# hjr37/diff-gaussian-rasterization

Measured on AMD Instinct MI355X. Metric: Mviews/sec fwd+bwd @1080p, 500k Gaussians, higher is better.
Workload: dtype f32

## Files before the change

### diff-gaussian-rasterization_amd/csrc/render_common.h

```cpp
#pragma once
#include "dgr_common.h"
#include "kernels.h"
#include "wave_reduce.h"
#include "exact_math.h"

namespace dgr {

__device__ __forceinline__ uint4 blend_slot(const uint4* __restrict__ sched, const uint2* __restrict__ ranges,
                                            const uint32_t* __restrict__ sched_flag, int tiles, bool* overflowed = nullptr,
                                            bool* quadrant_lists = nullptr) {
    const int flag = __builtin_amdgcn_readfirstlane((int)*sched_flag);
    if (overflowed) *overflowed = (flag & 2) != 0;
    if (quadrant_lists) *quadrant_lists = (flag & 4) != 0;
    if (flag & 1) return sched[blockIdx.x];
    const int tile = xcd_contiguous((int)blockIdx.x, tiles);
    const uint2 r = ranges[tile];
    return make_uint4((uint32_t)tile, r.x, r.y, 0u);
}

__device__ __forceinline__ bool wave_any(bool p) { return __builtin_amdgcn_ballot_w64(p) != 0ull; }

namespace {

constexpr float LOG2E = 1.4426950408889634f, LN2 = 0.6931471805599453f;
constexpr float ALPHA_MIN = 15.0f / 255.0f;

enum { ALPHA_REF = 0, ALPHA_FAST = 1, ALPHA_GLIBC = 2 };
template <int AM>
struct AlphaPath {
    static constexpr bool LOG2 = (AM == ALPHA_FAST);
    static constexpr float PSCALE = LOG2 ? LOG2E : 1.0f;
    static constexpr float PUNSCALE = LOG2 ? LN2 : 1.0f;
    static constexpr bool TABLE = (AM == ALPHA_GLIBC);
};
template <int AM, bool UNTESTED_ARG = false>
__device__ __forceinline__ float alpha_raw(float o, float p2, const uint64_t* tab) {
    if (AM == ALPHA_FAST) return o * __builtin_amdgcn_exp2f(p2);
    if (AM == ALPHA_GLIBC) return o * exp_glibc<UNTESTED_ARG>(p2, tab);
    return o * exp_p32<UNTESTED_ARG>(p2);
}
template <int AM>
__device__ __forceinline__ float t_div(float T, float om, float& inv) {
    if (AM == ALPHA_FAST) { inv = __builtin_amdgcn_rcpf(om); return T * inv; }
    return div_ref(T, om, inv);
}

template <int NB, typename LIST_T = unsigned short, int NLISTS = 4, bool KEEP_ID = true>
struct StagedT {
    typedef LIST_T list_t;
    static constexpr bool HAS_ID = KEEP_ID;
    static constexpr int SLOTS = NB;
    static constexpr int SENTINEL = NB;
    static constexpr int LIST_LD = NB + 8;
    static constexpr int REC_BYTES = 32;
    float4 rec[2 * (NB + 1)];
    float4 rgbd[NB + 1];
    uint32_t id[KEEP_ID ? NB : 1];
    LIST_T list[NLISTS][LIST_LD];
    int cnt4[4][NLISTS];
};
using Staged = StagedT<DGR_TILE_PIX>;

template <int AM>
__device__ __forceinline__ void gather_record(const float4* __restrict__ rec, uint32_t gid, float4& staged0, float4& q0, float4& q1, float4& q2) {
    constexpr float PSCALE = AlphaPath<AM>::PSCALE;
    q0 = rec[DGR_REC_STRIDE * (size_t)gid + 0];
    q1 = rec[DGR_REC_STRIDE * (size_t)gid + 1];
    q2 = rec[DGR_REC_STRIDE * (size_t)gid + 2];
    staged0 = make_float4(q0.x, q0.y, -0.5f * PSCALE * q1.x, -0.5f * PSCALE * q1.z);
}

template <bool HALF_CODES>
__device__ __forceinline__ unsigned reach_code(const float4& q0, const float4& q1, float l2, float tile_x0, float tile_y0);

template <int AM, bool HALF_CODES = false, class S>
__device__ __forceinline__ unsigned stage_one(S& s, int slot, uint32_t gid, const float4* __restrict__ rec,
                                              float tile_x0, float tile_y0) {
    float4 q0, q1, q2;
    gather_record<AM>(rec, gid, s.rec[2 * slot], q0, q1, q2);
    const float o = q0.w;
    const float l2 = __log2f(o * (255.0f / 15.0f));
    constexpr float PSCALE = AlphaPath<AM>::PSCALE;
    float lthr = (o > 0.f) ? (-l2 * (AlphaPath<AM>::LOG2 ? 1.0f : LN2) - 1.0e-4f) : 3.0e38f;
    float zword = __int_as_float(slot);
    if (HALF_CODES) {
        lthr = fmaxf(lthr, -3.0e38f);
        lthr = __int_as_float(((__float_as_int(lthr) + 0xFF) & ~0xFF) | slot);
        zword = 0.f;
    }
    s.rec[2 * slot + 1] = make_float4(-PSCALE * q1.y, o, zword, lthr);
    s.rgbd[slot] = make_float4(q2.x, q2.y, q2.z, q0.z);
    if (S::HAS_ID) s.id[slot] = gid;
    return reach_code<HALF_CODES>(q0, q1, l2, tile_x0, tile_y0);
}
template <bool HALF_CODES>
__device__ __forceinline__ unsigned reach_code(const float4& q0, const float4& q1, float l2, float tile_x0, float tile_y0) {
    const float tau = 2.0f * 0.6931471805599453f * l2;
    const float det = q1.x * q1.z - q1.y * q1.y;
    if (!(tau > 0.0f)) return 0u;
    if (!(det > 0.0f && q1.x > 0.0f && q1.z > 0.0f)) return HALF_CODES ? 0xFFu : 0xFu;
    const float k = tau * __builtin_amdgcn_rcpf(det);
    const float hx = __builtin_amdgcn_sqrtf(k * q1.z) * 1.001f + 0.05f, hy = __builtin_amdgcn_sqrtf(k * q1.x) * 1.001f + 0.05f;
    const float gx = q0.x - tile_x0, gy = q0.y - tile_y0;
    const bool xl = (gx + hx >= 0.0f) && (gx - hx <= 7.0f), xr = (gx + hx >= 8.0f) && (gx - hx <= 15.0f);
    if (HALF_CODES) {
        const float lo = gy - hy, hi = gy + hy;
        const unsigned xm = (xl ? 0x33u : 0u) | (xr ? 0xCCu : 0u);
        const unsigned ym = ((hi >= 0.0f) && (lo <= 3.0f) ? 0x05u : 0u) | ((hi >= 4.0f) && (lo <= 7.0f) ? 0x0Au : 0u) |
                            ((hi >= 8.0f) && (lo <= 11.0f) ? 0x50u : 0u) | ((hi >= 12.0f) && (lo <= 15.0f) ? 0xA0u : 0u);
        return xm & ym;
    }
    const bool yt = (gy + hy >= 0.0f) && (gy - hy <= 7.0f), yb = (gy + hy >= 8.0f) && (gy - hy <= 15.0f);
    return (xl && yt ? 1u : 0u) | (xr && yt ? 2u : 0u) | (xl && yb ? 4u : 0u) | (xr && yb ? 8u : 0u);
}

constexpr int TAG_SHIFT = DGR_TAG_SHIFT;
constexpr uint32_t ID_MASK = DGR_ID_MASK;
enum { TAGS_BYTES_QUADRANT = 1, TAGS_BYTES_HALVES = 2 };

__device__ __forceinline__ uint8_t* half_tags(const uint32_t* point_list, const uint32_t* sched_flag) {
    return carve_binning(reinterpret_cast<char*>(const_cast<uint32_t*>(point_list)), (size_t)sched_flag[-1]).pair_cov;
}
__device__ __forceinline__ uint32_t spread4(uint32_t c) { return (c & 1u) | ((c & 2u) << 1) | ((c & 4u) << 2) | ((c & 8u) << 3); }
__device__ __forceinline__ uint32_t fold8(uint32_t t) {
    t = (t | (t >> 1)) & 0x55u;
    return (t & 1u) | ((t >> 1) & 2u) | ((t >> 2) & 4u) | ((t >> 3) & 8u);
}

__device__ __forceinline__ uint32_t pack4(uint32_t w) { return (w & 1u) | ((w >> 7) & 2u) | ((w >> 14) & 4u) | ((w >> 21) & 8u); }
__device__ __forceinline__ uint32_t tag_byte(uint32_t up, uint32_t lo) { return spread4(pack4(up)) | (spread4(pack4(lo)) << 1); }

template <int AM, int TAGS, class S>
__device__ __forceinline__ unsigned stage_tagged(S& s, int slot, uint32_t entry, const float4* __restrict__ rec,
                                                 const uint8_t* __restrict__ tag8) {
    constexpr float PSCALE = AlphaPath<AM>::PSCALE;
    unsigned code = (unsigned)*tag8;
    if (code == 0u) return 0u;
    if (TAGS == TAGS_BYTES_QUADRANT) code = fold8(code);
    const uint32_t gid = entry & ID_MASK;
    float4 q0, q1, q2;
    gather_record<AM>(rec, gid, s.rec[2 * slot], q0, q1, q2);
    s.rec[2 * slot + 1] = make_float4(-PSCALE * q1.y, q0.w, __int_as_float(slot * 4), __int_as_float(slot * 16));
    s.rgbd[slot] = make_float4(q2.x, q2.y, q2.z, q0.z);
    s.id[slot] = gid;
    return code;
}

__device__ __forceinline__ uint2* live_list(const uint32_t* point_list, const uint32_t* sched_flag) {
    return reinterpret_cast<uint2*>(carve_binning(reinterpret_cast<char*>(const_cast<uint32_t*>(point_list)), (size_t)sched_flag[-1]).pair_keys);
}

template <int NB, int NLISTS = 4>
struct StagedLiveT {
    typedef uint32_t list_t;
    static constexpr bool HAS_ID = true;
    static constexpr int SLOTS = NB;
    static constexpr int SENTINEL = NB;
    static constexpr int LIST_LD = NB + 8;
    static constexpr int REC_BYTES = 48;
    float4 rec[3 * (NB + 1)];
    uint32_t id[NB];
    uint32_t list[NLISTS][LIST_LD];
    int cnt4[4][NLISTS];
};

template <int AM, bool QUADRANT, class S>
__device__ __forceinline__ unsigned stage_live(S& s, int slot, uint2 e, const float4* __restrict__ rec) {
    constexpr float PSCALE = AlphaPath<AM>::PSCALE;
    unsigned code = e.y & 0xFFu;
    if (QUADRANT) code = fold8(code);
    const uint32_t gid = e.x & ID_MASK;
    float4 q0, q1, q2;
    gather_record<AM>(rec, gid, s.rec[3 * slot], q0, q1, q2);
    s.rec[3 * slot + 1] = make_float4(-PSCALE * q1.y, q0.w, __int_as_float(slot * 4), __int_as_float((int)(e.y >> 8)));
    s.rec[3 * slot + 2] = make_float4(q2.x, q2.y, q2.z, q0.z);
    s.id[slot] = gid;
    return code;
}
template <class S>
__device__ __forceinline__ void write_sentinel_live(S& s) {
    constexpr int NB = S::SLOTS;
    s.rec[3 * NB] = make_float4(0.f, 0.f, 0.f, 0.f);
    s.rec[3 * NB + 1] = make_float4(0.f, 0.f, __int_as_float(NB * 4), __int_as_float(0x7fffffff));
    s.rec[3 * NB + 2] = make_float4(0.f, 0.f, 0.f, 0.f);
}

__device__ __forceinline__ int lanes_below(unsigned long long m) {
    return (int)__builtin_amdgcn_mbcnt_hi((unsigned)(m >> 32), __builtin_amdgcn_mbcnt_lo((unsigned)m, 0u));
}

template <class S>
__device__ __forceinline__ int build_lists(S& s, unsigned code, int tid, int wave, int lane) {
    typedef typename S::list_t LT;
    unsigned long long bal[4];
#pragma unroll
    for (int w = 0; w < 4; w++) {
        bal[w] = __ballot((code >> w) & 1u);
        if (lane == 0) s.cnt4[wave][w] = __popcll(bal[w]);
    }
    __syncthreads();
#pragma unroll
    for (int w = 0; w < 4; w++) {
        if ((code >> w) & 1u) {
            int base = 0;
            for (int sw = 0; sw < wave; sw++) base += s.cnt4[sw][w];
            s.list[w][base + lanes_below(bal[w])] = (LT)(tid * S::REC_BYTES);
        }
    }
    const int n = __builtin_amdgcn_readfirstlane(s.cnt4[0][wave] + s.cnt4[1][wave] + s.cnt4[2][wave] + s.cnt4[3][wave]);
    __syncthreads();
    if (lane < 4) s.list[wave][n + lane] = (LT)(S::SENTINEL * S::REC_BYTES);
    return n;
}

template <class S>
__device__ __forceinline__ int build_half_lists(S& s, unsigned code, int tid, int wave, int lane) {
    typedef typename S::list_t LT;
    unsigned long long bal[8];
#pragma unroll
    for (int l = 0; l < 8; l++) {
        bal[l] = __ballot((code >> l) & 1u);
        if (lane == 0) s.cnt4[wave][l] = __popcll(bal[l]);
    }
    __syncthreads();
    int before = 0, all = 0;
    if (lane < 8) {
#pragma unroll
        for (int sw = 0; sw < 4; sw++) {
            const int c = s.cnt4[sw][lane];
            before += sw < wave ? c : 0;
            all += c;
        }
    }
#pragma unroll
    for (int l = 0; l < 8; l++) {
        const int base = __builtin_amdgcn_readlane(before, l);
        if ((code >> l) & 1u) s.list[l][base + lanes_below(bal[l])] = (LT)(tid * S::REC_BYTES);
    }
    const int l0 = 2 * wave;
    const int n0 = __builtin_amdgcn_readlane(all, l0), n1 = __builtin_amdgcn_readlane(all, l0 + 1);
    __syncthreads();
    const int n = max(n0, n1);
    for (int i = n0 + lane; i < n + 4; i += 64) s.list[l0][i] = (LT)(S::SENTINEL * S::REC_BYTES);
    for (int i = n1 + lane; i < n + 4; i += 64) s.list[l0 + 1][i] = (LT)(S::SENTINEL * S::REC_BYTES);
    return n;
}

template <class S>
__device__ __forceinline__ int build_paired_lists(S& s, unsigned code8, int tid, int wave, int lane, unsigned long long (&split)[2]) {
    typedef typename S::list_t LT;
    static_assert(sizeof(LT) == 4 && S::SLOTS <= 128, "paired lists: 32-bit entries, at most two ranks per lane");
    unsigned long long bal[4];
#pragma unroll
    for (int w = 0; w < 4; w++) {
        bal[w] = __ballot(((code8 >> (2 * w)) & 3u) != 0u);
        if (lane == 0) s.cnt4[wave][w] = __popcll(bal[w]);
    }
    __syncthreads();
    int before = 0, all = 0;
    if (lane < 4) {
#pragma unroll
        for (int sw = 0; sw < 4; sw++) {
            const int c = s.cnt4[sw][lane];
            before += sw < wave ? c : 0;
            all += c;
        }
    }
#pragma unroll
    for (int w = 0; w < 4; w++) {
        const unsigned t = (code8 >> (2 * w)) & 3u;
        const int base = __builtin_amdgcn_readlane(before, w);
        if (t != 0u) s.list[2 * w][base + lanes_below(bal[w])] = (LT)(tid * S::REC_BYTES) | t;
    }
    const int n = __builtin_amdgcn_readlane(all, wave);
    __syncthreads();
    LT* const LU = s.list[2 * wave];
    LT* const LL = s.list[2 * wave + 1];
    if (n <= 64) {
        const bool have = lane < n;
        const unsigned e0 = have ? LU[lane] : 0u;
        const int t0 = (int)(e0 & 3u);
        const int tm1 = __builtin_amdgcn_update_dpp(0, t0, 0x138, 0xf, 0xf, true);
        const int tm2 = __builtin_amdgcn_update_dpp(0, tm1, 0x138, 0xf, 0xf, true);
        const int tp1 = __builtin_amdgcn_update_dpp(0, t0, 0x130, 0xf, 0xf, true);
        const int tp2 = __builtin_amdgcn_update_dpp(0, tp1, 0x130, 0xf, 0xf, true);
        const bool odd = (lane & 1) != 0;
        const bool a_self = odd ? (tm1 * t0 == 2) : (t0 * tp1 == 2);
        const bool a_side = odd ? (tp1 * tp2 == 2) : (tm2 * tm1 == 2);
        const bool p2 = !a_self && !a_side && (odd ? (t0 * tp1 == 2) : (tm1 * t0 == 2));
        const bool first = odd ? p2 : a_self, second = odd ? a_self : p2;
        const unsigned long long keep = __ballot(have && !second);
        const int steps = __popcll(keep);
        if (have) {
            const int st = lanes_below(keep) - (second ? 1 : 0);
            const LT o = e0 & ~3u;
            if (first || second) {
                (t0 == 1 ? LU : LL)[st] = o;
            } else {
                LU[st] = o;
                LL[st] = o;
            }
        }
        if (lane < 4) {
            LU[steps + lane] = (LT)(S::SENTINEL * S::REC_BYTES);
            LL[steps + lane] = (LT)(S::SENTINEL * S::REC_BYTES);
        }
        split[0] = __ballot(lane < steps && LU[lane] != LL[lane]);
        split[1] = 0ull;
        return steps;
    }
    const LT ea = lane < n ? LU[lane] : 0u, eb = lane + 64 < n ? LU[lane + 64] : 0u;
    if (lane < n) { LU[lane] = ea & ~3u; LL[lane] = ea & ~3u; }
    if (lane + 64 < n) { LU[lane + 64] = eb & ~3u; LL[lane + 64] = eb & ~3u; }
    if (lane < 4) {
        LU[n + lane] = (LT)(S::SENTINEL * S::REC_BYTES);
        LL[n + lane] = (LT)(S::SENTINEL * S::REC_BYTES);
    }
    split[0] = split[1] = 0ull;
    return n;
}
// ... 159 lines not shown
```

### diff-gaussian-rasterization_amd/csrc/render_light.hip

```cpp
#include "render_common.h"

namespace dgr {
namespace {

constexpr int FWD_UNROLL = 2;

template <bool HALVES>
struct StagedFwd {
    typedef StagedT<DGR_TILE_PIX, unsigned short, HALVES ? 8 : 4, !HALVES> staged_t;
    staged_t f;
    float unc[DGR_TILE_PIX];
    uint32_t cnt[DGR_TILE_PIX];
    uint32_t hit[DGR_TILE_PIX];
    alignas(16) uint32_t live4[4];
    uint64_t exptab[32];
};

template <class SF>
__device__ __forceinline__ uint32_t flush_slot(SF& sf, const RenderFwdLightArgs& a, uint8_t* tag8, uint2* live, uint32_t list0, uint32_t pos0,
                                               uint32_t live_base, int tid, bool staged) {
    uint32_t t8 = 0u;
    if (staged) {
        if constexpr (!SF::staged_t::HAS_ID) {
            t8 = tag_byte(sf.hit[tid], __float_as_uint(sf.f.rec[2 * tid + 1].z));
        } else {
            t8 = spread4(pack4(sf.hit[tid])) * 3u;
        }
        tag8[list0 + pos0 + tid] = (uint8_t)t8;
    }
    const unsigned long long bal = __ballot(t8 != 0u);
    if ((tid & 63) == 0) sf.live4[tid >> 6] = (uint32_t)__popcll(bal);
    __syncthreads();
    const uint4 c = *reinterpret_cast<const uint4*>(sf.live4);
    if (t8 != 0u) {
        const int wave = tid >> 6;
        const uint32_t before = (wave > 0 ? c.x : 0u) + (wave > 1 ? c.y : 0u) + (wave > 2 ? c.z : 0u);
        uint32_t gid;
        if constexpr (SF::staged_t::HAS_ID) gid = sf.f.id[tid];
        else gid = a.point_list[list0 + pos0 + tid];
        live[list0 + live_base + before + (uint32_t)lanes_below(bal)] = make_uint2(gid, ((pos0 + (uint32_t)tid) << 8) | t8);
        if (sf.cnt[tid] != 0u) {
            atomicAdd(&a.gau_uncertainty[gid], sf.unc[tid]);
            atomicAdd(&a.gau_related_pixels[gid], (int)sf.cnt[tid]);
        }
    }
    return live_base + (uint32_t)__builtin_amdgcn_readfirstlane((int)(c.x + c.y + c.z + c.w));
}

template <int AM, bool HALVES>
__device__ __forceinline__ void render_fwd_light_body(const RenderFwdLightArgs& a, StagedFwd<HALVES>& sf, const uint4 slot, const bool overflowed) {
    typename StagedFwd<HALVES>::staged_t& s = sf.f;
    const int tile = (int)slot.x;
    const int tid = threadIdx.x, wave = tid >> 6, lane = tid & 63;
    const auto [tx, ty, px, py, inside, pix_id] = tile_pixel(tile, a.grid_x, a.W, a.H, wave, lane);
    const f2 pxy = {(float)px, (float)py};
    const float tile_x0 = (float)(tx * DGR_BLOCK_X), tile_y0 = (float)(ty * DGR_BLOCK_Y);
    const int my_list = HALVES ? 2 * wave + (lane >> 5) : wave;
    uint8_t* const tag8 = half_tags(a.point_list, a.sched_flag);
    uint2* const live = live_list(a.point_list, a.sched_flag);
    uint32_t live_base = 0;
    unsigned char* const mark_base = (HALVES && lane >= 32) ? reinterpret_cast<unsigned char*>(&s.rec[1].z) + wave
                                                             : reinterpret_cast<unsigned char*>(sf.hit) + wave;
    const int mark_stride = (HALVES && lane >= 32) ? 32 : 4;

    const uint2 range = make_uint2(slot.y, slot.z);
    const int total = (int)(range.y - range.x);

    float T = 1.0f, C0 = 0.f, C1 = 0.f, C2 = 0.f, weight = 0.f, Dd = 0.f, D_median = 0.f;
    uint32_t last_contributor = 0;
    float ub = inside ? 0.f : -__builtin_inff();
    const float gt_px = inside ? a.gt_depth[pix_id] : 0.f;
    if (tid == 0) write_sentinel(s);
    if (AlphaPath<AM>::TABLE) exp_ref_table_fill(sf.exptab, tid);
    bool have_flush = false;
    int last_base = 0;

    for (int base = 0; base < total; base += DGR_TILE_PIX) {
        if (__syncthreads_and(ub < 0.f)) break;
        last_base = base;
        if (have_flush) live_base = flush_slot(sf, a, tag8, live, range.x, (uint32_t)(base - DGR_TILE_PIX), live_base, tid, true);
        sf.unc[tid] = 0.f;
        sf.cnt[tid] = 0u;
        sf.hit[tid] = 0u;
        have_flush = true;
        const int cnt = min(DGR_TILE_PIX, total - base);
        unsigned code = 0;
        if (tid < cnt) code = stage_one<AM, HALVES>(s, tid, a.point_list[range.x + base + tid], a.rec, tile_x0, tile_y0);
        const int n = HALVES ? build_half_lists(s, code, tid, wave, lane) : build_lists(s, code, tid, wave, lane);

        for (int k = 0; k < n; k += FWD_UNROLL) {
            float4 q0[FWD_UNROLL], q1[FWD_UNROLL];
            load2(s, my_list, k, q0, q1);
#pragma unroll
            for (int u = 0; u < FWD_UNROLL; u++) {
                f2 dxy;
                const float p2 = pair_p2<AM>(q0[u], q1[u], pxy, dxy);
                if ((p2 <= ub) & (p2 >= q1[u].w)) {
                  const float alpha = fminf(0.99f, alpha_raw<AM>(q1[u].y, p2, sf.exptab));
                  if (alpha >= ALPHA_MIN) {
#pragma clang fp contract(off)
                    const float test_T = T * (1.0f - alpha);
                    if (test_T < 0.0001f) {
                        ub = -__builtin_inff();
                    } else {
                        const int j = HALVES ? (__float_as_int(q1[u].w) & 0xFF) : __float_as_int(q1[u].z);
                        const float4 cd = s.rgbd[j];
                        mark_base[j * mark_stride] = 1;
                        const float w = alpha * T;
                        C0 = __builtin_fmaf(cd.x, w, C0); C1 = __builtin_fmaf(cd.y, w, C1); C2 = __builtin_fmaf(cd.z, w, C2);
                        weight = weight + w;
                        Dd = __builtin_fmaf(cd.w, w, Dd);
                        if (T > 0.5f && test_T < 0.5f) {
                            D_median = cd.w;
                            const float e = cd.w - gt_px;
                            atomicAdd(&sf.unc[j], e * e * w);
                            atomicAdd(&sf.cnt[j], 1u);
                        }
                        T = test_T;
                        last_contributor = (uint32_t)(base + j + 1);
                    }
                  }
                }
            }
            if (!wave_any(ub >= 0.f)) break;
        }
    }
    __syncthreads();
    if (have_flush) live_base = flush_slot(sf, a, tag8, live, range.x, (uint32_t)last_base, live_base, tid, tid < total - last_base);
    if (tid == 0) a.live_counts[tile] = live_base;
    for (int p = (have_flush ? last_base + DGR_TILE_PIX : 0) + tid; p < total; p += DGR_TILE_PIX) tag8[range.x + p] = 0;

    if (overflowed) {
        C0 = C1 = C2 = weight = Dd = D_median = __builtin_nanf("");
    }
    if (inside) {
        const uint32_t N = (uint32_t)a.W * (uint32_t)a.H;
        a.n_contrib[pix_id] = last_contributor;
        a.out_color[pix_id] = C0 + T * a.bg[0];
        a.out_color[N + pix_id] = C1 + T * a.bg[1];
        a.out_color[2 * N + pix_id] = C2 + T * a.bg[2];
        a.out_alpha[pix_id] = weight;
        a.out_depth[pix_id] = Dd;
        a.out_median[pix_id] = D_median;
        a.out_depth_var[pix_id] = 0.0f;
    }
}

template <int AM>
__global__ void __launch_bounds__(256, 8) render_fwd_light_kernel(RenderFwdLightArgs a) {
    __shared__ union { StagedFwd<true> h; StagedFwd<false> q; } sf;
    if (a.rep.host && blockIdx.x == 0 && threadIdx.x == 0) report_status(a.rep, a.status);
    bool overflowed, quadrant_lists;
    const uint4 slot = blend_slot(a.sched, a.ranges, a.sched_flag, a.grid_x * a.grid_y, &overflowed, &quadrant_lists);
    if (quadrant_lists) render_fwd_light_body<AM, false>(a, sf.q, slot, overflowed);
    else render_fwd_light_body<AM, true>(a, sf.h, slot, overflowed);
}

constexpr int NACC_LIGHT = 14;

struct BwdTailLight {
    uint64_t exptab[32];
};
template <bool DET, bool HALVES = false, bool ABS = false>
using StagedBwd = BwdBatch<StagedLiveT<bwd_batch_entries(DET), HALVES ? 8 : 4>, NACC_LIGHT, DET, ABS, BwdTailLight>;

template <int AM, bool DO_MAP, bool DO_POSE, bool DET, bool LEAN, bool HALVES, bool ABS = false>
__device__ __forceinline__ void render_bwd_light_body(const RenderBwdLightArgs& a, StagedBwd<DET, HALVES, ABS>& sb, const uint4 slot,
                                                      float* __restrict__ abs_out = nullptr) {
    static_assert(!HALVES || !DET, "half-wave / paired lists: not with the deterministic kernel's planes (LDS)");
    static_assert(!ABS || (DO_MAP && !DET), "absgrad: the mapping backward, not the deterministic kernel");
    constexpr bool PAIRED = HALVES && DO_MAP;
    typedef StagedBwd<DET, HALVES, ABS> SB;
    constexpr int BWD_NB = SB::NB, BWD_LD = SB::LD;
    typename SB::staged_t& s = sb.f;
    const int tile = (int)slot.x;
    const int tid = threadIdx.x, wave = tid >> 6, lane = tid & 63;
    const auto [tx, ty, px, py, inside, pix_id] = tile_pixel(tile, a.grid_x, a.W, a.H, wave, lane);
    const uint32_t N = (uint32_t)a.W * (uint32_t)a.H;
    const float pxf = (float)px, pyf = (float)py;
    const f2 pxy = {pxf, pyf};

    const int total = __builtin_amdgcn_readfirstlane((int)a.live_counts[tile]);
    if (total <= 0) return;
    const uint2* const live = live_list(a.point_list, a.sched_flag) + slot.y;
    const int last_contributor = inside ? (int)a.n_contrib[pix_id] : 0;

    if (tid == 0) write_sentinel_live(s);
    if (AlphaPath<AM>::TABLE) exp_ref_table_fill(sb.t.exptab, tid);

    const float T_final = inside ? (1.0f - a.alphas[pix_id]) : 0.f;
    float T = T_final;
    float dpix0 = 0.f, dpix1 = 0.f, dpix2 = 0.f, dpix_depth = 0.f, dpix_median = 0.f, dpix_var = 0.f, gt_px = 0.f, dpix_sil = 0.f;
    if (inside) {
        dpix0 = __builtin_nontemporal_load(a.dL_dpix + pix_id);
        dpix1 = __builtin_nontemporal_load(a.dL_dpix + N + pix_id);
        dpix2 = __builtin_nontemporal_load(a.dL_dpix + 2 * N + pix_id);
        dpix_depth = __builtin_nontemporal_load(a.dL_dpix_depth + pix_id);
        if (a.dL_dpix_silhouette) dpix_sil = __builtin_nontemporal_load(a.dL_dpix_silhouette + pix_id);
        if (!LEAN) {
            if (a.dL_dpix_median) dpix_median = __builtin_nontemporal_load(a.dL_dpix_median + pix_id);
            if (a.dL_dpix_var) dpix_var = __builtin_nontemporal_load(a.dL_dpix_var + pix_id);
            gt_px = __builtin_nontemporal_load(a.gt_depth + pix_id);
        }
    }
    const float bg_term = -T_final * ((a.bg[0] * dpix0 + a.bg[1] * dpix1 + a.bg[2] * dpix2) - dpix_sil);
    const float ddelx_dx = 0.5f * a.W, ddely_dy = 0.5f * a.H;
    float S = 0.f;
    float mid_thr = 0.5f;
    int my_comp;
    if (DO_MAP) {
        const int c = (lane >= 48) ? 12 : wave_reduce12d_comp(lane);
        my_comp = ((lane & 3) != 0 || c > 11) ? -1 : (c == 10 ? (DO_POSE ? 13 : 10) : c == 11 ? (DO_POSE ? 10 : -1) : c);
    } else if (HALVES) {
        const int c = half_reduce3_comp(lane);
        my_comp = c == 0 ? 4 : c == 1 ? 5 : c == 2 ? 13 : -1;
    } else {
        const int c = wave_reduce4_comp(lane);
        my_comp = ((lane & 15) == 0 && c < 3) ? (c == 0 ? 4 : c == 1 ? 5 : 13) : -1;
    }
    const int my_list = HALVES ? 2 * wave + (lane >> 5) : wave;

    float* const my_acc = sb.acc + (DET ? wave * SB::PLANE : 0) + (my_comp >= 0 ? my_comp : 0) * BWD_LD;

    for (int hi = total; hi > 0; hi -= BWD_NB) {
        const int lo = max(0, hi - BWD_NB);
        const int cnt = hi - lo;
        __syncthreads();
        unsigned code = 0;
        if (tid < cnt) code = stage_live<AM, !HALVES>(s, tid, live[lo + tid], a.rec);
        if (!DET) clear_acc(sb, tid);
        unsigned long long split[2] = {0ull, 0ull};
        const int n = PAIRED   ? build_paired_lists(s, code, tid, wave, lane, split)
                      : HALVES ? build_half_lists(s, code, tid, wave, lane)
                               : build_lists(s, code, tid, wave, lane);

        constexpr int U = PAIRED ? 1 : 2;
        for (int k = ((n + U - 1) / U) * U - U; k >= 0; k -= U) {
            float4 q0[2], q1[2];
            unsigned off[2];
            if (U == 2) {
                const uint2 pk = *reinterpret_cast<const uint2*>(&s.list[my_list][k]);
                off[0] = pk.x;
                off[1] = pk.y;
            } else {
                off[0] = off[1] = s.list[my_list][k];
            }
#pragma unroll
            for (int u = 0; u < U; u++) {
                q0[u] = *reinterpret_cast<const float4*>(reinterpret_cast<const char*>(s.rec) + off[u]);
                q1[u] = *reinterpret_cast<const float4*>(reinterpret_cast<const char*>(s.rec) + off[u] + 16);
            }
#pragma unroll
            for (int u = U - 1; u >= 0; u--) {
                f2 dxy;
                const float p2 = pair_p2<AM>(q0[u], q1[u], pxy, dxy);
                const float dx = dxy.x, dy = dxy.y;
                const int j4 = __float_as_int(q1[u].z);
                const float oG = alpha_raw<AM, true>(q1[u].y, p2, sb.t.exptab);
                const bool valid = (__float_as_int(q1[u].w) < last_contributor) & (p2 <= 0.0f) & !(oG < ALPHA_MIN);
                const float oGm = valid ? oG : 0.f;
                const float alpha = fminf(0.99f, oGm);
                const float4 cd = *reinterpret_cast<const float4*>(reinterpret_cast<const char*>(s.rec) + off[u] + 32);
                const float om = 1.f - alpha;
                float inv;
                T = t_div<AM>(T, om, inv);
                const float w = alpha * T;
                const float e = cd.w - gt_px;
                const float X = LEAN ? cd.x * dpix0 + cd.y * dpix1 + cd.z * dpix2 + cd.w * dpix_depth
                                     : cd.x * dpix0 + cd.y * dpix1 + cd.z * dpix2 + cd.w * dpix_depth + (e * e) * dpix_var;
                const float dL_dalpha = (X - S) * T + bg_term * inv;
                S = alpha * X + om * S;
                const float qq = oGm * dL_dalpha;
                const float qdx = qq * dx, qdy = qq * dy;
                const float wd = w * dpix_depth;
                float tot;
                if (DO_MAP) {
                    float gmed = 0.f;
                    if (!LEAN) {
                        const bool fire = valid & (T > mid_thr);
                        gmed = fire ? dpix_median : 0.f;
                        mid_thr = fire ? __builtin_inff() : mid_thr;
                    }
                    float g[12];
                    g[0] = w * dpix0;
                    g[1] = w * dpix1;
                    g[2] = w * dpix2;
                    g[3] = LEAN ? wd : wd + 2.f * ((dpix_var * w) * e);
                    g[4] = qdx;
                    g[5] = qdy;
                    g[6] = qdx * dx;
                    g[7] = qdx * dy;
                    g[8] = qdy * dy;
                    g[9] = qq;
                    g[10] = DO_POSE ? wd : gmed;
                    g[11] = DO_POSE ? gmed : 0.f;
                    if (ABS) abs_pair_terms<AM, NACC_LIGHT, BWD_LD>(sb.acc, q0[u], q1[u], qdx, qdy, j4, lane);
                    if (PAIRED) {
                        float u0, u1;
                        wave_reduce12d_head(g, u0, u1);
                        const int st = k + u;
                        if ((split[st >> 6] >> (st & 63)) & 1ull) {
                            const float r0 = quad_sum(u0), r1 = quad_sum(u1);
                            auto comp_of = [](int slot) { return slot < 10 ? slot : slot == 10 ? (DO_POSE ? 13 : 10) : (DO_POSE ? 10 : -1); };
                            const int s1 = wave_reduce12d_half_slot1(lane);
                            const int c0 = (lane & 3) == 0 ? comp_of(wave_reduce12d_half_slot0(lane)) : -1;
                            const int c1 = ((lane & 3) == 0 && s1 >= 0) ? comp_of(s1) : -1;
                            deliver_pair<BWD_LD>(sb.acc, j4, c0, c1, r0, r1);
                            continue;
                        }
                        tot = wave_reduce12d_tail(u0, u1);
                    } else {
                        tot = wave_reduce12d(g);
                    }
                } else if (HALVES) {
                    tot = half_reduce3(qdx, qdy, wd);
                } else {
                    float g4[4] = {qdx, qdy, wd, 0.f};
                    tot = wave_reduce4(g4);
                }
                if (my_comp >= 0) {
                    float* const cell = reinterpret_cast<float*>(reinterpret_cast<char*>(my_acc) + j4);
                    if (DET) *cell = tot; else atomicAdd(cell, tot);
                }
            }
        }

        __syncthreads();
        if (DET && tid < BWD_NB) {
            uint32_t row = ~0u;
            if (code != 0u) {
                det_fold_planes<NACC_LIGHT, SB::PLANE, BWD_LD>(sb.acc, code, tid, [](int k) {
                    return DO_MAP ? (k <= 9 || k == 10 || (DO_POSE && k == 13)) : (k == 4 || k == 5 || k == 13);
                });
                row = det_row_of(a.det_rect, a.det_goff, s.id[tid], tx, ty);
            }
            sb.inst[tid] = row;
        }
        if (DET) __syncthreads();
        if (code != 0u) {
            const float4 r0 = s.rec[3 * tid], r1 = s.rec[3 * tid + 1];
            mean2d_from_moments(unscaled_conic<AM>(r0, r1), sb.acc[4 * BWD_LD + tid], sb.acc[5 * BWD_LD + tid], ddelx_dx, ddely_dy);
            if (ABS) abs_flush<NACC_LIGHT, BWD_LD>(sb.acc, s.id, tid, ddelx_dx, ddely_dy, abs_out);
            if (DO_MAP) {
                sb.acc[6 * BWD_LD + tid] *= -0.5f;
                sb.acc[7 * BWD_LD + tid] *= -0.5f;
                sb.acc[8 * BWD_LD + tid] *= -0.5f;
                sb.acc[9 * BWD_LD + tid] *= __builtin_amdgcn_rcpf(r1.y);
            }
        }
        __syncthreads();
        if (DET) {
            det_store_rows<NACC_LIGHT, BWD_LD>(sb.acc, sb.inst, cnt, a.det_rows, a.det_R, tid);
        } else {
            flush_acc<NACC_LIGHT, BWD_LD>(sb.acc, s.id, cnt, a.acc, tid);
        }
    }
}

template <int AM, bool DO_POSE, bool LEAN, bool BY_FRAME>
__global__ void __launch_bounds__(256, LEAN ? 8 : 7) render_bwd_light_abs_kernel(RenderBwdLightArgs a, float* abs_out) {
    __shared__ union { StagedBwd<false, BY_FRAME, true> h; StagedBwd<false, false, true> q; } sb;
    bool quadrant_lists = true;
    const uint4 slot = blend_slot(a.sched, a.ranges, a.sched_flag, a.grid_x * a.grid_y, nullptr, BY_FRAME ? &quadrant_lists : nullptr);
    if (BY_FRAME && !quadrant_lists) render_bwd_light_body<AM, true, DO_POSE, false, LEAN, BY_FRAME, true>(a, sb.h, slot, abs_out);
    else render_bwd_light_body<AM, true, DO_POSE, false, LEAN, false, true>(a, sb.q, slot, abs_out);
}

template <int AM, bool DO_MAP, bool DO_POSE, bool DET = false, bool LEAN = false, bool BY_FRAME = false>
__global__ void __launch_bounds__(256, 8) render_bwd_light_kernel(RenderBwdLightArgs a) {
    static_assert(!BY_FRAME || !DET, "the deterministic kernel walks quadrant lists");
    __shared__ union { StagedBwd<DET, BY_FRAME> h; StagedBwd<DET, false> q; } sb;
    bool quadrant_lists = true;
    const uint4 slot = blend_slot(a.sched, a.ranges, a.sched_flag, a.grid_x * a.grid_y, nullptr, BY_FRAME ? &quadrant_lists : nullptr);
    if (BY_FRAME && !quadrant_lists) render_bwd_light_body<AM, DO_MAP, DO_POSE, DET, LEAN, BY_FRAME>(a, sb.h, slot);
    else render_bwd_light_body<AM, DO_MAP, DO_POSE, DET, LEAN, false>(a, sb.q, slot);
}

__device__ __forceinline__ uint32_t rect_tiles(ushort4 r) { return (r.z > r.x && r.w > r.y) ? (uint32_t)(r.z - r.x) * (uint32_t)(r.w - r.y) : 0u; }
__global__ void __launch_bounds__(256) det_block_sums_kernel(int P, const ushort4* __restrict__ rect, uint32_t* __restrict__ blk) {
    __shared__ uint32_t red[4];
    const int g = blockIdx.x * 256 + threadIdx.x;
    uint32_t v = g < P ? rect_tiles(rect[g]) : 0u;
#pragma unroll
    for (int off = 32; off > 0; off >>= 1) v += __shfl_xor(v, off, 64);
    if ((threadIdx.x & 63) == 0) red[threadIdx.x >> 6] = v;
    __syncthreads();
    if (threadIdx.x == 0) blk[blockIdx.x] = red[0] + red[1] + red[2] + red[3];
}
__global__ void __launch_bounds__(256) det_offsets_kernel(int P, const ushort4* __restrict__ rect, const uint32_t* __restrict__ blk,
                                                          uint32_t* __restrict__ goff) {
    __shared__ uint32_t red[4], wsum[4];
    uint32_t before = 0;
    for (int b = threadIdx.x; b < (int)blockIdx.x; b += 256) before += blk[b];
#pragma unroll
    for (int off = 32; off > 0; off >>= 1) before += __shfl_xor(before, off, 64);
    if ((threadIdx.x & 63) == 0) red[threadIdx.x >> 6] = before;
    const int g = blockIdx.x * 256 + threadIdx.x;
    const uint32_t n = g < P ? rect_tiles(rect[g]) : 0u;
    uint32_t incl = n;
#pragma unroll
    for (int off = 1; off < 64; off <<= 1) {
        const uint32_t v = __shfl_up(incl, off, 64);
        if ((threadIdx.x & 63) >= off) incl += v;
    }
    if ((threadIdx.x & 63) == 63) wsum[threadIdx.x >> 6] = incl;
    __syncthreads();
    uint32_t base = red[0] + red[1] + red[2] + red[3];
    for (int w = 0; w < (int)(threadIdx.x >> 6); w++) base += wsum[w];
    if (g < P) goff[g] = base + incl - n;
}
__global__ void __launch_bounds__(256) det_gather_kernel(int P, const ushort4* __restrict__ rect, const uint32_t* __restrict__ goff,
                                                         const float* __restrict__ rows, uint32_t R, float* __restrict__ acc) {
    const int g = blockIdx.x * 16 + (threadIdx.x >> 4), comp = threadIdx.x & 15;
    if (g >= P) return;
    uint32_t n = rect_tiles(rect[g]);
    if (n == 0u) return;
    const uint32_t first = goff[g];
    if (first >= R || n > R - first) {
        acc[(size_t)g * DGR_ACC_STRIDE + comp] = __builtin_nanf("");
        return;
    }
    const float* r = rows + (size_t)first * DGR_ACC_STRIDE + comp;
    float v = 0.f;
    for (uint32_t i = 0; i < n; i++) v += r[(size_t)i * DGR_ACC_STRIDE];
    acc[(size_t)g * DGR_ACC_STRIDE + comp] = v;
}

template <class F>
void with_map_pose(const RenderBwdLightArgs& a, F&& f) {
    if (!a.map_off && !a.track_off) f(std::true_type(), std::true_type());
    else if (!a.map_off) f(std::true_type(), std::false_type());
    else f(std::false_type(), std::true_type());
}
template <int AM, bool DET, bool LEAN, bool BY_FRAME>
void launch_bwd_light_instance(const RenderBwdLightArgs& a, int tiles, hipStream_t stream) {
    with_map_pose(a, [&](auto do_map, auto do_pose) {
        launch_blend((render_bwd_light_kernel<AM, decltype(do_map)::value, decltype(do_pose)::value, DET, LEAN, BY_FRAME>), dim3(tiles), dim3(256), stream, a);
    });
}
template <int AM, bool LEAN>
void launch_bwd_light_abs_instance(const RenderBwdLightArgs& a, float* abs_out, int tiles, hipStream_t stream) {
    with_map_pose(a, [&](auto, auto do_pose) {
        launch_blend((render_bwd_light_abs_kernel<AM, decltype(do_pose)::value, LEAN, true>), dim3(tiles), dim3(256), stream, a, abs_out);
    });
}

template <int AM>
void launch_bwd_light_mode(const RenderBwdLightArgs& a, int tiles, hipStream_t stream) {
    constexpr bool BF = AM != ALPHA_GLIBC;
    if (AM == ALPHA_REF && a.det_rows) launch_bwd_light_instance<ALPHA_REF, true, false, false>(a, tiles, stream);
    else if (AM == ALPHA_REF && !a.dL_dpix_median && !a.dL_dpix_var) launch_bwd_light_instance<ALPHA_REF, false, true, true>(a, tiles, stream);
    else launch_bwd_light_instance<AM, false, false, BF>(a, tiles, stream);
}
}

hipError_t launch_render_fwd_light(const RenderFwdLightArgs& a, int alpha_mode, hipStream_t stream) {
    const int tiles = a.grid_x * a.grid_y;
    if (tiles <= 0) return hipSuccess;
    switch (alpha_mode) {
        case ALPHA_FAST: launch_blend(render_fwd_light_kernel<ALPHA_FAST>, dim3(tiles), dim3(256), stream, a); break;
        case ALPHA_GLIBC: launch_blend(render_fwd_light_kernel<ALPHA_GLIBC>, dim3(tiles), dim3(256), stream, a); break;
        default: launch_blend(render_fwd_light_kernel<ALPHA_REF>, dim3(tiles), dim3(256), stream, a);
    }
    return hipGetLastError();
}
hipError_t launch_render_bwd_light(const RenderBwdLightArgs& a, int alpha_mode, hipStream_t stream) {
    const int tiles = a.grid_x * a.grid_y;
    if (tiles <= 0 || (a.track_off && a.map_off)) return hipSuccess;
    switch (alpha_mode) {
        case ALPHA_FAST: launch_bwd_light_mode<ALPHA_FAST>(a, tiles, stream); break;
        case ALPHA_GLIBC: launch_bwd_light_mode<ALPHA_GLIBC>(a, tiles, stream); break;
        default: launch_bwd_light_mode<ALPHA_REF>(a, tiles, stream);
    }
    return hipGetLastError();
}
hipError_t launch_render_bwd_light_abs(const RenderBwdLightArgs& a, float* dL_dmean2D_abs, int alpha_mode, hipStream_t stream) {
    const int tiles = a.grid_x * a.grid_y;
    if (tiles <= 0 || a.map_off) return hipSuccess;
    const bool lean = !a.dL_dpix_median && !a.dL_dpix_var;
    if (alpha_mode == ALPHA_FAST) launch_bwd_light_abs_instance<ALPHA_FAST, false>(a, dL_dmean2D_abs, tiles, stream);
    else if (alpha_mode == ALPHA_REF && lean) launch_bwd_light_abs_instance<ALPHA_REF, true>(a, dL_dmean2D_abs, tiles, stream);
    else if (alpha_mode == ALPHA_REF) launch_bwd_light_abs_instance<ALPHA_REF, false>(a, dL_dmean2D_abs, tiles, stream);
    else return hipErrorInvalidValue;
    return hipGetLastError();
}
namespace {
__global__ void __launch_bounds__(256) zero_floats_kernel(float* dst, size_t n) {
    const size_t stride = (size_t)gridDim.x * 256;
    for (size_t i = (size_t)blockIdx.x * 256 + threadIdx.x; i < n; i += stride) dst[i] = 0.f;
}
}
hipError_t launch_zero_floats(float* dst, size_t n, hipStream_t stream) {
    if (n == 0) return hipSuccess;
    const unsigned blocks = (unsigned)std::min<size_t>((n + 255) / 256, 256 * 16);
    launch(zero_floats_kernel, dim3(blocks), dim3(256), stream, dst, n);
    return hipGetLastError();
}
hipError_t launch_det_offsets(int P, const ushort4* rect, uint32_t* blk, uint32_t* goff, hipStream_t stream) {
    if (P <= 0) return hipSuccess;
    const int nb = (P + 255) / 256;
    launch(det_block_sums_kernel, dim3(nb), dim3(256), stream, P, rect, blk);
    launch(det_offsets_kernel, dim3(nb), dim3(256), stream, P, rect, (const uint32_t*)blk, goff);
    return hipGetLastError();
}
hipError_t launch_det_gather(int P, const ushort4* rect, const uint32_t* goff, const float* rows, uint32_t R, float* acc, hipStream_t stream) {
    if (P <= 0) return hipSuccess;
    launch(det_gather_kernel, dim3((P + 15) / 16), dim3(256), stream, P, rect, goff, rows, R, acc);
    return hipGetLastError();
}
}
```

Before: 0.002685.

## Restructure light forward flush loop and cut register pressure in blend kernels

```diff
diff --git a/diff-gaussian-rasterization_amd/csrc/render_common.h b/diff-gaussian-rasterization_amd/csrc/render_common.h
--- a/diff-gaussian-rasterization_amd/csrc/render_common.h
+++ b/diff-gaussian-rasterization_amd/csrc/render_common.h
@@ -3,19 +3,45 @@
 #include "kernels.h"
 #include "wave_reduce.h"
 #include "exact_math.h"
+#include <type_traits>
 
 namespace dgr {
 
+enum { BLEND_FLAG_SCHEDULE = 1, BLEND_FLAG_OVERFLOWED = 2, BLEND_FLAG_QUADRANT_LISTS = 4 };
+__device__ __forceinline__ int blend_flags(const uint32_t* __restrict__ sched_flag) { return __builtin_amdgcn_readfirstlane((int)*sched_flag); }
+__device__ __forceinline__ uint4 blend_slot(int flag, const uint4* __restrict__ sched, const uint2* __restrict__ ranges, int tiles) {
+    if (flag & BLEND_FLAG_SCHEDULE) return sched[blockIdx.x];
+    const int tile = xcd_contiguous((int)blockIdx.x, tiles);
+    const uint2 r = ranges[tile];
+    return make_uint4((uint32_t)tile, r.x, r.y, 0u);
+}
 __device__ __forceinline__ uint4 blend_slot(const uint4* __restrict__ sched, const uint2* __restrict__ ranges,
                                             const uint32_t* __restrict__ sched_flag, int tiles, bool* overflowed = nullptr,
                                             bool* quadrant_lists = nullptr) {
-    const int flag = __builtin_amdgcn_readfirstlane((int)*sched_flag);
-    if (overflowed) *overflowed = (flag & 2) != 0;
-    if (quadrant_lists) *quadrant_lists = (flag & 4) != 0;
-    if (flag & 1) return sched[blockIdx.x];
-    const int tile = xcd_contiguous((int)blockIdx.x, tiles);
-    const uint2 r = ranges[tile];
-    return make_uint4((uint32_t)tile, r.x, r.y, 0u);
+    const int flag = blend_flags(sched_flag);
+    if (overflowed) *overflowed = (flag & BLEND_FLAG_OVERFLOWED) != 0;
+    if (quadrant_lists) *quadrant_lists = (flag & BLEND_FLAG_QUADRANT_LISTS) != 0;
+    return blend_slot(flag, sched, ranges, tiles);
+}
+
+template <class T>
+__device__ __forceinline__ T& at_byte(T* base, uint32_t byte_off) {
+    return *reinterpret_cast<T*>(reinterpret_cast<char*>(const_cast<std::remove_const_t<T>*>(base)) + byte_off);
+}
+
+#define DGR_GLOBAL __attribute__((address_space(1)))
+template <class T>
+__device__ __forceinline__ T DGR_GLOBAL* global_at(T* uniform_ptr, uint32_t byte_off) {
+    asm volatile("" : "+s"(uniform_ptr));
+    return (T DGR_GLOBAL*)((char DGR_GLOBAL*)uniform_ptr + byte_off);
+}
+
+template <class ARGS>
+__device__ __forceinline__ const ARGS __attribute__((address_space(4)))* late_kernel_args() {
+    typedef const ARGS __attribute__((address_space(4)))* P;
+    P p = (P)__builtin_amdgcn_kernarg_segment_ptr();
+    asm volatile("" : "+s"(p));
+    return p;
 }
 
 __device__ __forceinline__ bool wave_any(bool p) { return __builtin_amdgcn_ballot_w64(p) != 0ull; }
diff --git a/diff-gaussian-rasterization_amd/csrc/render_light.hip b/diff-gaussian-rasterization_amd/csrc/render_light.hip
--- a/diff-gaussian-rasterization_amd/csrc/render_light.hip
+++ b/diff-gaussian-rasterization_amd/csrc/render_light.hip
@@ -7,7 +7,8 @@
 
 template <bool HALVES>
 struct StagedFwd {
-    typedef StagedT<DGR_TILE_PIX, unsigned short, HALVES ? 8 : 4, !HALVES> staged_t;
+    typedef StagedT<DGR_TILE_PIX, unsigned short, HALVES ? 8 : 4, false> staged_t;
+    static constexpr bool HALF_LISTS = HALVES;
     staged_t f;
     float unc[DGR_TILE_PIX];
     uint32_t cnt[DGR_TILE_PIX];
@@ -18,37 +19,35 @@
 
 template <class SF>
 __device__ __forceinline__ uint32_t flush_slot(SF& sf, const RenderFwdLightArgs& a, uint8_t* tag8, uint2* live, uint32_t list0, uint32_t pos0,
-                                               uint32_t live_base, int tid, bool staged) {
+                                               uint32_t live_base, int tid, bool staged, uint32_t gid, bool my_done, bool& all_done) {
     uint32_t t8 = 0u;
     if (staged) {
-        if constexpr (!SF::staged_t::HAS_ID) {
+        if constexpr (SF::HALF_LISTS) {
             t8 = tag_byte(sf.hit[tid], __float_as_uint(sf.f.rec[2 * tid + 1].z));
         } else {
             t8 = spread4(pack4(sf.hit[tid])) * 3u;
         }
-        tag8[list0 + pos0 + tid] = (uint8_t)t8;
+        *global_at(tag8 + (size_t)(list0 + pos0), (uint32_t)tid) = (uint8_t)t8;
     }
     const unsigned long long bal = __ballot(t8 != 0u);
     if ((tid & 63) == 0) sf.live4[tid >> 6] = (uint32_t)__popcll(bal);
-    __syncthreads();
+    all_done = __syncthreads_and(my_done);
     const uint4 c = *reinterpret_cast<const uint4*>(sf.live4);
     if (t8 != 0u) {
         const int wave = tid >> 6;
         const uint32_t before = (wave > 0 ? c.x : 0u) + (wave > 1 ? c.y : 0u) + (wave > 2 ? c.z : 0u);
-        uint32_t gid;
-        if constexpr (SF::staged_t::HAS_ID) gid = sf.f.id[tid];
-        else gid = a.point_list[list0 + pos0 + tid];
-        live[list0 + live_base + before + (uint32_t)lanes_below(bal)] = make_uint2(gid, ((pos0 + (uint32_t)tid) << 8) | t8);
+        *global_at(reinterpret_cast<unsigned long long*>(live + (size_t)(list0 + live_base)), (before + (uint32_t)lanes_below(bal)) * 8u) =
+            (unsigned long long)gid | ((unsigned long long)(((pos0 + (uint32_t)tid) << 8) | t8) << 32);
         if (sf.cnt[tid] != 0u) {
-            atomicAdd(&a.gau_uncertainty[gid], sf.unc[tid]);
-            atomicAdd(&a.gau_related_pixels[gid], (int)sf.cnt[tid]);
+            atomicAdd(&at_byte(a.gau_uncertainty, gid * 4u), sf.unc[tid]);
+            atomicAdd(&at_byte(a.gau_related_pixels, gid * 4u), (int)sf.cnt[tid]);
         }
     }
     return live_base + (uint32_t)__builtin_amdgcn_readfirstlane((int)(c.x + c.y + c.z + c.w));
 }
 
 template <int AM, bool HALVES>
-__device__ __forceinline__ void render_fwd_light_body(const RenderFwdLightArgs& a, StagedFwd<HALVES>& sf, const uint4 slot, const bool overflowed) {
+__device__ __forceinline__ void render_fwd_light_body(const RenderFwdLightArgs& a, StagedFwd<HALVES>& sf, const uint4 slot, const int frame_flags) {
     typename StagedFwd<HALVES>::staged_t& s = sf.f;
     const int tile = (int)slot.x;
     const int tid = threadIdx.x, wave = tid >> 6, lane = tid & 63;
@@ -59,6 +58,7 @@
     uint8_t* const tag8 = half_tags(a.point_list, a.sched_flag);
     uint2* const live = live_list(a.point_list, a.sched_flag);
     uint32_t live_base = 0;
+    uint32_t my_gid = 0;
     unsigned char* const mark_base = (HALVES && lane >= 32) ? reinterpret_cast<unsigned char*>(&s.rec[1].z) + wave
                                                              : reinterpret_cast<unsigned char*>(sf.hit) + wave;
     const int mark_stride = (HALVES && lane >= 32) ? 32 : 4;
@@ -69,23 +69,21 @@
     float T = 1.0f, C0 = 0.f, C1 = 0.f, C2 = 0.f, weight = 0.f, Dd = 0.f, D_median = 0.f;
     uint32_t last_contributor = 0;
     float ub = inside ? 0.f : -__builtin_inff();
-    const float gt_px = inside ? a.gt_depth[pix_id] : 0.f;
+    const float gt_px = inside ? at_byte(a.gt_depth, pix_id * 4u) : 0.f;
     if (tid == 0) write_sentinel(s);
     if (AlphaPath<AM>::TABLE) exp_ref_table_fill(sf.exptab, tid);
-    bool have_flush = false;
-    int last_base = 0;
-
-    for (int base = 0; base < total; base += DGR_TILE_PIX) {
-        if (__syncthreads_and(ub < 0.f)) break;
-        last_base = base;
-        if (have_flush) live_base = flush_slot(sf, a, tag8, live, range.x, (uint32_t)(base - DGR_TILE_PIX), live_base, tid, true);
+
+    int base = 0;
+    while (base < total) {
         sf.unc[tid] = 0.f;
         sf.cnt[tid] = 0u;
         sf.hit[tid] = 0u;
-        have_flush = true;
-        const int cnt = min(DGR_TILE_PIX, total - base);
+        const int cnt = total - base;
         unsigned code = 0;
-        if (tid < cnt) code = stage_one<AM, HALVES>(s, tid, a.point_list[range.x + base + tid], a.rec, tile_x0, tile_y0);
+        if (tid < cnt) {
+            my_gid = *global_at(a.point_list + (size_t)(range.x + (uint32_t)base), (uint32_t)tid * 4u);
+            code = stage_one<AM, HALVES>(s, tid, my_gid, a.rec, tile_x0, tile_y0);
+        }
         const int n = HALVES ? build_half_lists(s, code, tid, wave, lane) : build_lists(s, code, tid, wave, lane);
 
         for (int k = 0; k < n; k += FWD_UNROLL) {
@@ -124,25 +122,34 @@
             }
             if (!wave_any(ub >= 0.f)) break;
         }
-    }
-    __syncthreads();
-    if (have_flush) live_base = flush_slot(sf, a, tag8, live, range.x, (uint32_t)last_base, live_base, tid, tid < total - last_base);
-    if (tid == 0) a.live_counts[tile] = live_base;
-    for (int p = (have_flush ? last_base + DGR_TILE_PIX : 0) + tid; p < total; p += DGR_TILE_PIX) tag8[range.x + p] = 0;
-
-    if (overflowed) {
+        __syncthreads();
+        bool all_done;
+        live_base = flush_slot(sf, a, tag8, live, range.x, (uint32_t)base, live_base, tid, tid < cnt, my_gid, ub < 0.f, all_done);
+        base += DGR_TILE_PIX;
+        if (all_done) break;
+    }
+    if (tid == DGR_TILE_PIX - 1) a.live_counts[tile] = live_base;
+    for (int p = base + tid; p < total; p += DGR_TILE_PIX) at_byte(tag8 + (size_t)range.x, (uint32_t)p) = 0;
+
+    if (frame_flags & BLEND_FLAG_OVERFLOWED) {
         C0 = C1 = C2 = weight = Dd = D_median = __builtin_nanf("");
     }
     if (inside) {
-        const uint32_t N = (uint32_t)a.W * (uint32_t)a.H;
-        a.n_contrib[pix_id] = last_contributor;
-        a.out_color[pix_id] = C0 + T * a.bg[0];
-        a.out_color[N + pix_id] = C1 + T * a.bg[1];
-        a.out_color[2 * N + pix_id] = C2 + T * a.bg[2];
-        a.out_alpha[pix_id] = weight;
-        a.out_depth[pix_id] = Dd;
-        a.out_median[pix_id] = D_median;
-        a.out_depth_var[pix_id] = 0.0f;
+        const auto ka = late_kernel_args<RenderFwdLightArgs>();
+        const size_t N = (size_t)((uint32_t)a.W * (uint32_t)a.H);
+        float fx = pxy.x, fy = pxy.y;
+        asm volatile("" : "+v"(fx), "+v"(fy));
+        const uint32_t po = ((uint32_t)fy * (uint32_t)a.W + (uint32_t)fx) * 4u;
+        float* const out_color = ka->out_color;
+        const float* const bg = ka->bg;
+        at_byte(ka->n_contrib, po) = last_contributor;
+        at_byte(out_color, po) = C0 + T * bg[0];
+        at_byte(out_color + N, po) = C1 + T * bg[1];
+        at_byte(out_color + 2 * N, po) = C2 + T * bg[2];
+        at_byte(ka->out_alpha, po) = weight;
+        at_byte(ka->out_depth, po) = Dd;
+        at_byte(ka->out_median, po) = D_median;
+        at_byte(ka->out_depth_var, po) = 0.0f;
     }
 }
 
@@ -150,10 +157,10 @@
 __global__ void __launch_bounds__(256, 8) render_fwd_light_kernel(RenderFwdLightArgs a) {
     __shared__ union { StagedFwd<true> h; StagedFwd<false> q; } sf;
     if (a.rep.host && blockIdx.x == 0 && threadIdx.x == 0) report_status(a.rep, a.status);
-    bool overflowed, quadrant_lists;
-    const uint4 slot = blend_slot(a.sched, a.ranges, a.sched_flag, a.grid_x * a.grid_y, &overflowed, &quadrant_lists);
-    if (quadrant_lists) render_fwd_light_body<AM, false>(a, sf.q, slot, overflowed);
-    else render_fwd_light_body<AM, true>(a, sf.h, slot, overflowed);
+    const int frame_flags = blend_flags(a.sched_flag);
+    const uint4 slot = blend_slot(frame_flags, a.sched, a.ranges, a.grid_x * a.grid_y);
+    if (frame_flags & BLEND_FLAG_QUADRANT_LISTS) render_fwd_light_body<AM, false>(a, sf.q, slot, frame_flags);
+    else render_fwd_light_body<AM, true>(a, sf.h, slot, frame_flags);
 }
 
 constexpr int NACC_LIGHT = 14;
@@ -222,8 +229,13 @@
 
     float* const my_acc = sb.acc + (DET ? wave * SB::PLANE : 0) + (my_comp >= 0 ? my_comp : 0) * BWD_LD;
 
-    for (int hi = total; hi > 0; hi -= BWD_NB) {
-        const int lo = max(0, hi - BWD_NB);
+    int per = BWD_NB;
+    if (PAIRED && total > BWD_NB) {
+        const int nbatch = (total + BWD_NB - 1) / BWD_NB;
+        per = min(BWD_NB, (int)((float)total * __builtin_amdgcn_rcpf((float)nbatch)) + 1);
+    }
+    for (int hi = total; hi > 0; hi -= per) {
+        const int lo = max(0, hi - per);
         const int cnt = hi - lo;
         __syncthreads();
         unsigned code = 0;
diff --git a/profiles/asm_depth.py b/profiles/asm_depth.py
--- /dev/null
+++ b/profiles/asm_depth.py
@@ -0,0 +1,180 @@
+import collections
+import re
+import sys
+
+PAIR_MARKERS = ("ds_write_b8", "v_permlane32_swap")
+
+
+def kernels(lines):
+    out = []
+    for i, l in enumerate(lines):
+        m = re.match(r"^(_Z\w+):", l)
+        if m:
+            end = next((j for j in range(i, len(lines)) if lines[j].strip().startswith(".Lfunc_end")), None)
+            if end is not None:
+                out.append((m.group(1), i, end))
+    return out
+
+
+def metadata(lines, name):
+    meta = {}
+    idx = next((i for i, l in enumerate(lines) if l.strip() == ".name:           " + name or l.strip() == ".name: " + name
+                or re.match(r"^\s*\.name:\s+" + re.escape(name) + r"\s*$", l)), None)
+    if idx is None:
+        return meta
+    lo = idx
+    while lo > 0 and not lines[lo].lstrip().startswith("- ."):
+        lo -= 1
+    hi = idx + 1
+    while hi < len(lines) and not lines[hi].lstrip().startswith("- .") and not lines[hi].startswith("amdhsa."):
+        hi += 1
+    for l in lines[lo:hi]:
+        m = re.match(r"^\s*-?\s*\.(\w+):\s+(\S+)\s*$", l)
+        if m and m.group(1) in ("sgpr_count", "sgpr_spill_count", "vgpr_count", "vgpr_spill_count", "private_segment_fixed_size",
+                                "group_segment_fixed_size"):
+            meta[m.group(1)] = int(m.group(2))
+    return meta
+
+
+def classify(op):
+    if op.startswith("v_"):
+        return "valu"
+    if op.startswith("s_"):
+        return "salu"
+    if op.startswith("ds_"):
+        return "lds"
+    return "mem"
+
+
+class Region:
+    def __init__(self, title):
+        self.title = title
+        self.n = collections.Counter()
+        self.pair = False
+
+    def add(self, line):
+        op = line.split(";")[0].split()[0]
+        self.n[classify(op)] += 1
+        if op.startswith(("v_readlane", "v_writelane")):
+            self.n["lane"] += 1
+        if op.startswith(("v_mov_b32", "v_mov_b64", "v_accvgpr")):
+            self.n["mov"] += 1
+        if op.startswith("s_load") or op.startswith("s_buffer_load"):
+            self.n["sload"] += 1
+        if any(m in line for m in PAIR_MARKERS):
+            self.pair = True
+
+    def row(self):
+        n = self.n
+        return (f"{self.title:34s} valu {n['valu']:4d}  (v_mov {n['mov']:3d}, lane r/w {n['lane']:3d})   salu {n['salu']:4d} (s_load {n['sload']:2d})"
+                f"   lds {n['lds']:3d}   mem {n['mem']:3d}" + ("   <- pair loop" if self.pair else ""))
+
+
+def by_depth(lines, start, end):
+    body = lines[start + 1:end]
+    parent, depth_of = {}, {}
+    i = 0
+    blocks = []
+    while i < len(body):
+        l = body[i]
+        m = re.match(r"^(?:\.L(BB\d+_\d+)|; %bb\.\d+):(.*)", l)
+        if m:
+            label, comment = m.group(1), m.group(2)
+            j = i + 1
+            while j < len(body) and re.match(r"^\s+;", body[j]) and "implicit-def" not in body[j]:
+                comment += " " + body[j].strip()
+                j += 1
+            blocks.append((i, label, comment))
+            if label and "Loop Header" in comment:
+                d = int(re.search(r"Loop Header: Depth=(\d+)", comment).group(1))
+                depth_of[label] = d
+                ps = re.findall(r"Parent Loop (BB\d+_\d+) Depth=(\d+)", comment)
+                if ps:
+                    parent[label] = max(ps, key=lambda p: int(p[1]))[0]
+            i = j
+        else:
+            i += 1
+
+    def chain(h):
+        c = [h]
+        while c[0] in parent:
+            c.insert(0, parent[c[0]])
+        return c
+
+    regions, index = [], {}
+
+    def region(key, title):
+        if key not in index:
+            index[key] = Region(title)
+            regions.append(index[key])
+        return index[key]
+
+    nstraight = 0
+    cur = region(("straight", 0), "straight 0")
+    last_was_loop = False
+    bi = 0
+    for i, l in enumerate(body):
+        while bi < len(blocks) and blocks[bi][0] == i:
+            _, label, comment = blocks[bi]
+            bi += 1
+            hdr = None
+            if label and "Loop Header" in comment:
+                hdr = label
+            else:
+                m = re.search(r"in Loop: Header=(BB\d+_\d+) Depth=(\d+)", comment)
+                if m:
+                    hdr = m.group(1)
+            if hdr is None:
+                if last_was_loop:
+                    nstraight += 1
+                cur = region(("straight", nstraight), f"straight {nstraight}")
+                last_was_loop = False
+            else:
+                c = chain(hdr)
+                d = len(c)
+                title = ("  " * (d - 1)) + f"loop {c[-1]} depth {d}" + (f" (in {c[0]})" if d > 1 else "")
+                region(tuple(c[:1]), f"loop {c[0]} depth 1")
+                cur = region(tuple(c), title)
+                last_was_loop = True
+        if l.startswith("\t") and not l.strip().startswith((".", ";")) and l.split(";")[0].strip():
+            cur.add(l)
+    return regions
+
+
+def main():
+    path = sys.argv[1]
+    lines = open(path).read().splitlines()
+    if sys.argv[2] == "--all":
+        key = sys.argv[3] if len(sys.argv) > 3 else ""
+        for name, s, e in kernels(lines):
+            if key not in name:
+                continue
+            regs = by_depth(lines, s, e)
+            md = metadata(lines, name)
+            out_v = sum(r.n["valu"] for r in regs if not r.pair)
+            pair = [r.n["valu"] for r in regs if r.pair]
+            print(f"{name}\n    vgpr {md.get('vgpr_count')} sgpr {md.get('sgpr_count')} sgpr_spill {md.get('sgpr_spill_count')} vgpr_spill {md.get('vgpr_spill_count')}"
+                  f" scratch {md.get('private_segment_fixed_size')} lds {md.get('group_segment_fixed_size')}"
+                  f" | valu outside pair loops {out_v}, pair loops {pair}, lane r/w {sum(r.n['lane'] for r in regs)}, v_mov outside {sum(r.n['mov'] for r in regs if not r.pair)}")
+        return
+    key = sys.argv[2]
+    brief = "--brief" in sys.argv
+    for name, s, e in kernels(lines):
+        if key not in name:
+            continue
+        md = metadata(lines, name)
+        print(name)
+        print("  " + ", ".join(f"{k} {v}" for k, v in md.items()))
+        regs = by_depth(lines, s, e)
+        for r in regs:
+            if brief and sum(r.n.values()) == 0:
+                continue
+            print("  " + r.row())
+        tot = Region("total (static)")
+        for r in regs:
+            tot.n.update(r.n)
+        print("  " + tot.row())
+
+
+if __name__ == "__main__":
+    main()
```

After: 0.002720, median of 6. 1.01x the previous value.
